# rapidsai/wholegraph

Measured on AMD Instinct MI355X. Metric: gather_GBps_out (gathered output row bytes/s, reference gather_scatter_bench convention), higher is better.
Workload: dtype f32

## Files before the change

### wholegraph_amd/csrc/backend.hpp

```cpp
#pragma once

#include <cstddef>
#include <cstdint>

#include <wholememory/global_reference.h>
#include <wholememory/tensor_description.h>

extern "C" {

struct wm_rows_args {
  wholememory_gref_t gref;
  wholememory_dtype_t table_dtype;
  int64_t dim;
  int64_t table_stride;
  int64_t table_storage_offset;
  const void* indices;
  wholememory_dtype_t index_dtype;
  int64_t n;
  const void* row_map;
  void* plain;
  wholememory_dtype_t plain_dtype;
  int64_t plain_stride;
  int64_t plain_storage_offset;
  int max_blocks;
// ... 15 lines not shown

struct wm_optimizer_args {
  int type;
  const void* ids;
  wholememory_dtype_t index_dtype;
  const int32_t* run_starts;
  const int32_t* order;
  wholememory_dtype_t value_dtype;
  const void* grads;
  int64_t grad_stride;
  const void* self_grads;
  int64_t self_grad_stride;
  int64_t count;
  const int32_t* cache_slot_of;
  void* cache_data;
  uint8_t* cache_dirty;
  int64_t cache_row_elems;
  float* cache_state_data;
  int64_t cache_state_row_elems;
  void* local_table;
  int64_t table_stride;
  int64_t local_entry_offset;
  int64_t dim;
  float* per_element_state;
  int64_t per_element_stride;
  float* per_row_state;
  float weight_decay, epsilon, beta1, beta2, alpha, lr;
  int adam_w;
  void* long_run_ws;
  size_t long_run_ws_bytes;
  int fold_mode;
  int inputs_behind_sort;
};

struct wm_sample_args {
  wholememory_gref_t row_gref, col_gref;
  int64_t row_storage_offset, col_storage_offset;
  wholememory_dtype_t col_dtype;
  const int64_t* row_pairs;
  const void* centers;
  wholememory_dtype_t center_dtype;
  int n_center;
  int max_sample_count;
  uint64_t random_seed;
  const int* sample_offsets;
  void* out_ids;
  int* out_center_lid;
  int64_t* out_edge_gid;
  wholememory_gref_t weight_gref;
  int64_t weight_storage_offset;
  wholememory_dtype_t weight_dtype;
  const int* n_center_dev;
  void* fill_ff_ptr;
  size_t fill_ff_bytes;
};

struct wm_au_bounds {
  const int* n_target_dev;
  const int* n_neighbor_dev;
  int* n_unique_dev;
  int* publish_host_late;
  int table_is_clear;
  int pad_unique_tail;
};

struct wm_cache_args {
  int32_t* slot_of;
  int32_t* count;
  int64_t* row_of;
  uint8_t* dirty;
  char* data;
  int64_t cover_start;
  int64_t cover_rows;
  int64_t n_sets;
  int64_t set_cover;
  int64_t row_bytes;
  wholememory_gref_t raw_gref;
  int64_t raw_row_stride_bytes;
  int64_t raw_row_offset_bytes;
  char* data2;
  int64_t row_bytes2;
  wholememory_gref_t raw2_gref;
  int64_t raw2_row_stride_bytes;
};

struct wm_agg_args {
  const int32_t* row_ptr;
  const int32_t* col_ind;
  int64_t n_edges, n_dst, n_src, dim;
  int mean;
  const float* in;
  int64_t in_stride;
  const float* grad;
  int64_t grad_stride;
  float* out;
  int64_t out_stride;
};

struct wm_agg16_args {
  const int32_t* row_ptr;
  const int32_t* col_ind;
  int64_t n_edges, n_dst, n_src, dim;
  int mean;
  wholememory_dtype_t dtype;
  const void* in;
  int64_t in_stride;
  const void* grad;
  int64_t grad_stride;
  void* out;
  int64_t out_stride;
};

struct wm_gat_args {
  const int32_t* row_ptr;
  const int32_t* col_ind;
  int64_t n_edges, n_dst, n_src, heads, dim;
  float slope;
  int concat;
  const float* h;
  int64_t h_stride;
  const float* att;
  float* alpha;
  float* scores;
  float* out;
  int64_t out_stride;
  const float* grad;
  int64_t grad_stride;
  float* grad_h;
  int64_t grad_h_stride;
  float* grad_att;
};

struct wm_aggw_args {
  const int32_t* row_ptr;
  const int32_t* col_ind;
  const float* w;
  int64_t n_edges, n_dst, n_src, dim;
  int mean;
  const float* in;
  int64_t in_stride;
  const float* grad;
  int64_t grad_stride;
  float* out;
  int64_t out_stride;
  float* grad_w;
};

#define WM_MAX_EDGE_ATTRS 8
struct wm_edge_attr_args {
  const int64_t* edge_gid;
  const int* n_dev;
  int64_t n;
  int n_attrs;
  struct {
    wholememory_gref_t gref;
    int64_t storage_offset;
    int elt_bytes;
    void* out;
  } attr[WM_MAX_EDGE_ATTRS];
};

struct wm_gather_agg_args {
  wholememory_gref_t gref;
  wholememory_dtype_t table_dtype;
  int64_t table_rows;
  int64_t table_stride;
// ... 198 lines not shown
```

### wholegraph_amd/csrc/embedding_cache.cpp

```cpp
#include "embedding_cache.hpp"

#include <algorithm>
#include <cstring>

namespace wm {

row_cache::~row_cache()
{
  const auto* bk = backend();
  if (args.slot_of) bk->free_device(args.slot_of);
  if (args.count) bk->free_device(args.count);
  if (args.row_of) bk->free_device(args.row_of);
  if (args.dirty) bk->free_device(args.dirty);
  if (args.data) bk->free_device(args.data);
  if (args.data2) bk->free_device(args.data2);
  if (counters_dev) bk->free_device(counters_dev);
}

wholememory_error_code_t create_row_cache(row_cache** out, const wholememory_embedding_cache_policy_* policy,
                                          wholememory_tensor_t raw, wholememory_comm_t embedding_comm)
{
  const auto* bk = backend();
  if (bk->cache_update == nullptr) return WHOLEMEMORY_NOT_SUPPORTED;
  auto* desc = wholememory_tensor_get_tensor_description(raw);
  auto h     = wholememory_tensor_get_memory_handle(raw);
  std::unique_ptr<row_cache> c(new row_cache());
  c->same_comm = policy->cache_comm == embedding_comm;
  c->writable  = policy->access_type == WHOLEMEMORY_AT_READWRITE;
  c->dtype     = desc->dtype;
  c->row_elems = desc->strides[0];
  c->raw       = raw;
  const size_t es = wholememory_dtype_get_element_size(desc->dtype);
  auto& a         = c->args;
  a.row_bytes     = c->row_elems * static_cast<int64_t>(es);
  if (a.row_bytes % 16 != 0) return WHOLEMEMORY_LOGIC_ERROR;
  a.raw_row_stride_bytes = a.row_bytes;
  a.raw_row_offset_bytes = desc->storage_offset * static_cast<int64_t>(es);
  if (c->same_comm) {
    std::vector<size_t> off = entry_offsets_of(h, static_cast<size_t>(a.row_bytes));
    a.cover_start           = static_cast<int64_t>(off[embedding_comm->world_rank]);
    a.cover_rows            = static_cast<int64_t>(off[embedding_comm->world_rank + 1]) - a.cover_start;
    a.raw_gref              = local_shard_gref(h);
  } else {
    a.cover_start = 0;
    a.cover_rows  = desc->sizes[0];
    if (wholememory_get_memory_type(h) == WHOLEMEMORY_MT_DISTRIBUTED && embedding_comm->world_size > 1) {
      c->raw_addressable = false;
      a.raw_gref         = wholememory_create_continuous_global_reference(nullptr);
    } else {
      WHOLEMEMORY_RETURN_ON_FAIL(tensor_mapped_gref(raw, &a.raw_gref));
    }
  }
  if (a.cover_rows >= (INT64_C(1) << 31)) return WHOLEMEMORY_NOT_SUPPORTED;
  int64_t slots = static_cast<int64_t>(static_cast<double>(a.cover_rows) * policy->cache_ratio);
  slots         = std::min(a.cover_rows + 63, std::max<int64_t>(slots, a.cover_rows > 0 ? 64 : 0));
  a.n_sets      = (slots + 63) / 64;
  a.set_cover   = a.n_sets > 0 ? (a.cover_rows + a.n_sets - 1) / a.n_sets : 0;
  const int64_t n_slots = a.n_sets * 64;
  auto dev_alloc = [&](void** p, size_t bytes) { WM_BK(bk->malloc_device(p, std::max<size_t>(bytes, 16))); };
  dev_alloc(reinterpret_cast<void**>(&a.slot_of), sizeof(int32_t) * a.cover_rows);
  dev_alloc(reinterpret_cast<void**>(&a.count), sizeof(int32_t) * a.cover_rows);
  dev_alloc(reinterpret_cast<void**>(&a.row_of), sizeof(int64_t) * n_slots);
  dev_alloc(reinterpret_cast<void**>(&a.dirty), n_slots);
  dev_alloc(reinterpret_cast<void**>(&a.data), static_cast<size_t>(n_slots) * a.row_bytes);
  dev_alloc(reinterpret_cast<void**>(&c->counters_dev), 32);
  WM_BK(bk->memset_async(a.slot_of, 0xff, sizeof(int32_t) * a.cover_rows, nullptr));
  WM_BK(bk->memset_async(a.count, 0, sizeof(int32_t) * a.cover_rows, nullptr));
  WM_BK(bk->memset_async(a.row_of, 0xff, sizeof(int64_t) * n_slots, nullptr));
  WM_BK(bk->memset_async(a.dirty, 0, n_slots, nullptr));
  WM_BK(bk->memset_async(c->counters_dev, 0, 32, nullptr));
  WM_BK(bk->stream_sync(nullptr));
  *out = c.release();
  return WHOLEMEMORY_SUCCESS;
}

wholememory_error_code_t row_cache_update(row_cache* c, const void* ids, wholememory_dtype_t index_dtype, int64_t n,
                                          int64_t key_upper_bound, wholememory_env_func_t* env, void* stream)
{
  const auto* bk = backend();
  if (n == 0 || c->args.n_sets == 0) return WHOLEMEMORY_SUCCESS;
  if (n >= (INT64_C(1) << 31)) return WHOLEMEMORY_INVALID_INPUT;
  sorted_ids s(env);
  int rc = s.run(ids, index_dtype, n, key_upper_bound, 0, stream);
  if (rc != 0) return rc == -1 ? WHOLEMEMORY_INVALID_INPUT : WHOLEMEMORY_CUDA_ERROR;
  rc = bk->cache_update(&c->args, s.unique, index_dtype, s.starts, s.n_unique_dev, n, nullptr, nullptr, nullptr, stream);
  if (rc != 0) return rc == -1 ? WHOLEMEMORY_INVALID_INPUT : WHOLEMEMORY_CUDA_ERROR;
  WM_BK(bk->stream_sync(stream));
  return WHOLEMEMORY_SUCCESS;
}

wholememory_error_code_t row_cache_plan(row_cache* c, const void* ids, wholememory_dtype_t index_dtype, int64_t n, int64_t key_upper_bound,
                                        wholememory_env_func_t* env, void* stream, temp_mem* rows_mem, temp_mem* slots_mem,
                                        int64_t* n_fill)
{
  const auto* bk = backend();
  *n_fill        = 0;
  auto* fill_rows  = static_cast<int64_t*>(rows_mem->device(n, WHOLEMEMORY_DT_INT64));
  auto* fill_slots = static_cast<int64_t*>(slots_mem->device(n, WHOLEMEMORY_DT_INT64));
  if (n == 0 || c->args.n_sets == 0) return WHOLEMEMORY_SUCCESS;
  if (n >= (INT64_C(1) << 31) || c->writable) return WHOLEMEMORY_INVALID_INPUT;
  sorted_ids s(env);
  temp_mem count(env), host_n(env);
  auto* d_count = static_cast<int*>(count.device(1, WHOLEMEMORY_DT_INT));
  WM_BK(bk->memset_async(d_count, 0, sizeof(int), stream));
  int rc = s.run(ids, index_dtype, n, key_upper_bound, 0, stream);
  if (rc != 0) return rc == -1 ? WHOLEMEMORY_INVALID_INPUT : WHOLEMEMORY_CUDA_ERROR;
  rc = bk->cache_update(&c->args, s.unique, index_dtype, s.starts, s.n_unique_dev, n, fill_rows, fill_slots, d_count, stream);
  if (rc != 0) return rc == -1 ? WHOLEMEMORY_INVALID_INPUT : WHOLEMEMORY_CUDA_ERROR;
  auto* h = static_cast<int*>(host_n.pinned(1, WHOLEMEMORY_DT_INT));
  WM_BK(bk->memcpy_async(h, d_count, sizeof(int), stream));
  WM_BK(bk->stream_sync(stream));
  *n_fill = *h;
  return WHOLEMEMORY_SUCCESS;
}

wholememory_error_code_t row_cache_install(row_cache* c, const void* rows_data, const int64_t* slots, int64_t n_fill,
                                           void* stream)
{
  const auto* bk = backend();
  if (n_fill == 0) return WHOLEMEMORY_SUCCESS;
  wm_rows_args a{};
  a.gref          = wholememory_create_continuous_global_reference(c->args.data);
  a.table_dtype   = c->dtype;
  a.dim           = c->row_elems;
  a.table_stride  = c->row_elems;
  a.indices       = slots;
  a.index_dtype   = WHOLEMEMORY_DT_INT64;
  a.n             = n_fill;
  a.plain         = const_cast<void*>(rows_data);
  a.plain_dtype   = c->dtype;
  a.plain_stride  = c->row_elems;
  a.max_blocks    = -1;
  WM_BK(bk->scatter_rows(&a, stream));
  return WHOLEMEMORY_SUCCESS;
}

wholememory_error_code_t row_cache_split(row_cache* c, const void* ids, wholememory_dtype_t index_dtype, int64_t n,
                                         int64_t* cache_idx, void* raw_idx, void* stream)
{
  int rc = backend()->cache_split(&c->args, ids, index_dtype, n, cache_idx, raw_idx, c->counters_dev, stream);
  if (rc != 0) return rc == -1 ? WHOLEMEMORY_INVALID_INPUT : WHOLEMEMORY_CUDA_ERROR;
  c->lookups += n;
  return WHOLEMEMORY_SUCCESS;
}

wholememory_error_code_t row_cache_gather(row_cache* c, const wm_rows_args& a, wholememory_env_func_t* env, void* stream)
{
  const auto* bk = backend();
  if (a.n == 0) return WHOLEMEMORY_SUCCESS;
  temp_mem cache_idx_mem(env), raw_idx_mem(env);
  auto* cache_idx = static_cast<int64_t*>(cache_idx_mem.device(a.n, WHOLEMEMORY_DT_INT64));
  void* raw_idx   = raw_idx_mem.device(a.n, a.index_dtype);
  WHOLEMEMORY_RETURN_ON_FAIL(row_cache_split(c, a.indices, a.index_dtype, a.n, cache_idx, raw_idx, stream));
  wm_rows_args hit        = a;
  hit.gref                = wholememory_create_continuous_global_reference(c->args.data);
  hit.table_stride        = c->row_elems;
  hit.table_storage_offset = 0;
  hit.indices             = cache_idx;
  hit.index_dtype         = WHOLEMEMORY_DT_INT64;
  WM_BK(bk->gather_rows(&hit, stream));
  wm_rows_args miss = a;
  miss.indices      = raw_idx;
  WM_BK(bk->gather_rows(&miss, stream));
  WM_BK(bk->stream_sync(stream));
  return WHOLEMEMORY_SUCCESS;
}

wholememory_error_code_t row_cache_attach_states(row_cache* c, wholememory_tensor_t state_local)
{
  const auto* bk = backend();
  if (!c->same_comm || !c->writable || c->args.data2 != nullptr) return WHOLEMEMORY_INVALID_INPUT;
  WHOLEMEMORY_RETURN_ON_FAIL(row_cache_writeback(c, true, nullptr));
  auto* d = wholememory_tensor_get_tensor_description(state_local);
  if (d->dtype != WHOLEMEMORY_DT_FLOAT || d->dim != 2) return WHOLEMEMORY_INVALID_INPUT;
  auto& a                 = c->args;
  a.row_bytes2            = d->strides[0] * static_cast<int64_t>(sizeof(float));
  a.raw2_row_stride_bytes = a.row_bytes2;
  if (a.row_bytes2 % 16 != 0) return WHOLEMEMORY_LOGIC_ERROR;
  char* local = static_cast<char*>(wholememory_tensor_get_data_pointer(state_local));
  a.raw2_gref = wholememory_create_continuous_global_reference(local - a.cover_start * a.row_bytes2);
  void* p     = nullptr;
  WM_BK(bk->malloc_device(&p, std::max<size_t>(static_cast<size_t>(a.n_sets) * 64 * a.row_bytes2, 16)));
  a.data2 = static_cast<char*>(p);
  return WHOLEMEMORY_SUCCESS;
}

wholememory_error_code_t row_cache_writeback(row_cache* c, bool drop, void* stream)
{
  const auto* bk = backend();
  int rc         = bk->cache_writeback(&c->args, drop ? 1 : 0, stream);
  if (rc != 0) return WHOLEMEMORY_CUDA_ERROR;
  return bk->stream_sync(stream) == 0 ? WHOLEMEMORY_SUCCESS : WHOLEMEMORY_CUDA_ERROR;
}

wholememory_error_code_t row_cache_info(row_cache* c, int64_t* slots, int64_t* occupied, int64_t* dirty, int64_t* hits,
                                        int64_t* lookups, void* stream)
{
  const auto* bk = backend();
  if (bk->cache_info(&c->args, c->counters_dev + 1, stream) != 0) return WHOLEMEMORY_CUDA_ERROR;
  unsigned long long h[3] = {0, 0, 0};
  WM_BK(bk->memcpy_async(h, c->counters_dev, sizeof(h), stream));
  WM_BK(bk->stream_sync(stream));
  if (slots) *slots = c->args.n_sets * 64;
  if (occupied) *occupied = static_cast<int64_t>(h[1]);
  if (dirty) *dirty = static_cast<int64_t>(h[2]);
  if (hits) *hits = static_cast<int64_t>(h[0]);
  if (lookups) *lookups = c->lookups;
  return WHOLEMEMORY_SUCCESS;
}

}
```

### wholegraph_amd/csrc/embedding_cache.hpp

```cpp
#pragma once

#include <wholememory/embedding.h>

#include "backend.hpp"
#include "ops_internal.hpp"

struct wholememory_embedding_cache_policy_ {
  wholememory_comm_t cache_comm;
  wholememory_memory_type_t cache_memory_type;
  wholememory_memory_location_t cache_memory_location;
  wholememory_access_type_t access_type;
  float cache_ratio;
};

namespace wm {

struct row_cache {
  wm_cache_args args{};
  bool same_comm = false;
  bool writable  = false;
  bool raw_addressable = true;
  wholememory_tensor_t raw = nullptr;
  wholememory_dtype_t dtype = WHOLEMEMORY_DT_UNKNOWN;
  int64_t row_elems         = 0;
  unsigned long long* counters_dev = nullptr;
  int64_t lookups                  = 0;
  ~row_cache();
};

wholememory_error_code_t create_row_cache(row_cache** out, const wholememory_embedding_cache_policy_* policy,
                                          wholememory_tensor_t raw, wholememory_comm_t embedding_comm);

wholememory_error_code_t row_cache_update(row_cache* c, const void* ids, wholememory_dtype_t index_dtype, int64_t n,
                                          int64_t key_upper_bound, wholememory_env_func_t* env, void* stream);

wholememory_error_code_t row_cache_gather(row_cache* c, const wm_rows_args& a, wholememory_env_func_t* env, void* stream);

wholememory_error_code_t row_cache_plan(row_cache* c, const void* ids, wholememory_dtype_t index_dtype, int64_t n,
                                        int64_t key_upper_bound, wholememory_env_func_t* env, void* stream, temp_mem* rows_mem, temp_mem* slots_mem,
                                        int64_t* n_fill);
wholememory_error_code_t row_cache_install(row_cache* c, const void* rows_data, const int64_t* slots, int64_t n_fill,
                                           void* stream);
wholememory_error_code_t row_cache_split(row_cache* c, const void* ids, wholememory_dtype_t index_dtype, int64_t n,
                                         int64_t* cache_idx, void* raw_idx, void* stream);

wholememory_error_code_t row_cache_attach_states(row_cache* c, wholememory_tensor_t state_local);

wholememory_error_code_t row_cache_writeback(row_cache* c, bool drop, void* stream);
wholememory_error_code_t row_cache_info(row_cache* c, int64_t* slots, int64_t* occupied, int64_t* dirty, int64_t* hits,
                                        int64_t* lookups, void* stream);

}
```

### wholegraph_amd/csrc/kernels/cache.hip

```cpp
#include <hip/hip_runtime.h>
#include <stdint.h>

#include <algorithm>

#include "../backend.hpp"

namespace wm {
namespace {

constexpr int kBlock = 256;

struct raw_view {
  char* base;
  char* const* rank_ptrs;
  const size_t* rank_offsets;
  size_t chunk_stride;
  int world_size;
  int same_chunk;
  int64_t row_stride_bytes;
  int64_t row_offset_bytes;
};

struct raw2_view {
  char* base;
  int64_t row_stride_bytes;
};
inline raw2_view make_raw2(const wm_cache_args& c)
{
  return raw2_view{c.data2 != nullptr ? static_cast<char*>(c.raw2_gref.pointer) : nullptr, c.raw2_row_stride_bytes};
}

inline raw_view make_raw(const wm_cache_args& c)
{
  raw_view v{};
  v.chunk_stride = c.raw_gref.stride;
  v.world_size   = c.raw_gref.world_size;
  v.same_chunk   = c.raw_gref.same_chunk ? 1 : 0;
  if (c.raw_gref.stride == 0) {
    v.base = static_cast<char*>(c.raw_gref.pointer);
  } else {
    v.rank_ptrs    = static_cast<char* const*>(c.raw_gref.pointer);
    v.rank_offsets = c.raw_gref.rank_memory_offsets;
  }
  v.row_stride_bytes = c.raw_row_stride_bytes;
  v.row_offset_bytes = c.raw_row_offset_bytes;
  return v;
}

__device__ __forceinline__ char* raw_row(const raw_view& v, int64_t row)
{
  const size_t off = static_cast<size_t>(v.row_offset_bytes) + static_cast<size_t>(row) * static_cast<size_t>(v.row_stride_bytes);
  if (v.chunk_stride == 0) return v.base + off;
  int rank;
  size_t start;
  if (v.same_chunk) {
    rank  = static_cast<int>(off / v.chunk_stride);
    start = static_cast<size_t>(rank) * v.chunk_stride;
  } else {
    rank = 0;
    for (int r = 1; r < v.world_size; r++)
      if (off >= v.rank_offsets[r]) rank = r;
    start = v.rank_offsets[rank];
  }
  return v.rank_ptrs[rank] + (off - start);
}

__device__ __forceinline__ void wave_copy_row(char* dst, const char* src, int row_bytes, int lane)
{
  typedef uint32_t u32x4 __attribute__((ext_vector_type(4)));
  for (int o = lane * 16; o < row_bytes; o += 64 * 16) *reinterpret_cast<u32x4*>(dst + o) = *reinterpret_cast<const u32x4*>(src + o);
}

struct cache_dev {
  int32_t* slot_of;
  int32_t* count;
  int64_t* row_of;
  uint8_t* dirty;
  char* data;
  int64_t cover_start, cover_rows, n_sets, set_cover;
  int row_bytes;
  char* data2;
  int row_bytes2;
};

inline cache_dev make_dev(const wm_cache_args& c)
{
  return cache_dev{c.slot_of, c.count, c.row_of, c.dirty, c.data, c.cover_start, c.cover_rows, c.n_sets, c.set_cover,
                   static_cast<int>(c.row_bytes), c.data2, static_cast<int>(c.row_bytes2)};
}

template <typename IdxT>
__global__ void cache_count_kernel(cache_dev c, const IdxT* unique_rows, const int32_t* run_starts, const int64_t* n_unique)
{
  const int64_t u = static_cast<int64_t>(blockIdx.x) * blockDim.x + threadIdx.x;
  if (u >= *n_unique) return;
  const int64_t r = static_cast<int64_t>(unique_rows[u]) - c.cover_start;
  if (r < 0 || r >= c.cover_rows) return;
  c.count[r] += run_starts[u + 1] - run_starts[u];
}

struct fill_list {
  int64_t* rows;
  int64_t* slots;
  int* count;
};

template <typename IdxT>
__global__ __launch_bounds__(kBlock) void cache_update_kernel(cache_dev c, raw_view raw, raw2_view raw2,
                                                              const IdxT* unique_rows, const int64_t* n_unique_p,
                                                              fill_list fill)
{
  const int lane    = threadIdx.x & 63;
  const int64_t set = (static_cast<int64_t>(blockIdx.x) * kBlock + threadIdx.x) >> 6;
  if (set >= c.n_sets) return;
  const int64_t nu  = *n_unique_p;
  const int64_t lo_row = c.cover_start + set * c.set_cover;
  const int64_t hi_row = min(c.cover_start + c.cover_rows, lo_row + c.set_cover);
  auto lower = [&](int64_t key) {
    int64_t a = 0, b = nu;
    while (a < b) {
      const int64_t m = (a + b) >> 1;
      const IdxT v    = unique_rows[m];
      if (v >= 0 && static_cast<int64_t>(v) < key)
        a = m + 1;
      else
        b = m;
    }
    return a;
  };
  const int64_t first = lower(lo_row), last = lower(hi_row);
  if (first >= last) return;
  const int64_t slot  = set * 64 + lane;
  int64_t my_row      = c.row_of[slot];
  int32_t my_cnt      = my_row >= 0 ? c.count[my_row] : -1;
  for (int64_t j = first; j < last; j++) {
    const int64_t g = static_cast<int64_t>(unique_rows[j]);
    const int64_t r = g - c.cover_start;
    if (c.slot_of[r] >= 0) continue;
    const int32_t cand = c.count[r];
    uint64_t key = (static_cast<uint64_t>(static_cast<uint32_t>(my_cnt + 1)) << 8) | static_cast<uint32_t>(lane);
    for (int off = 32; off > 0; off >>= 1) {
      const uint64_t o = __shfl_xor(key, off, 64);
      key              = o < key ? o : key;
    }
    const int victim      = static_cast<int>(key & 0xff);
    const int32_t min_cnt = static_cast<int32_t>(key >> 8) - 1;
    if (cand <= min_cnt) continue;
    const int64_t vslot = set * 64 + victim;
    char* line          = c.data + vslot * c.row_bytes;
    const int64_t old   = __shfl(my_row, victim, 64);
    if (old >= 0) {
      if (fill.rows == nullptr && c.dirty[vslot]) {
        wave_copy_row(raw_row(raw, c.cover_start + old), line, c.row_bytes, lane);
        if (c.data2 != nullptr)
          wave_copy_row(raw2.base + (c.cover_start + old) * raw2.row_stride_bytes, c.data2 + vslot * c.row_bytes2, c.row_bytes2, lane);
      }
      if (lane == 0) c.slot_of[old] = -1;
    }
    if (fill.rows == nullptr) {
      wave_copy_row(line, raw_row(raw, g), c.row_bytes, lane);
      if (c.data2 != nullptr)
        wave_copy_row(c.data2 + vslot * c.row_bytes2, raw2.base + g * raw2.row_stride_bytes, c.row_bytes2, lane);
    } else if (lane == 0) {
      const int k   = atomicAdd(fill.count, 1);
      fill.rows[k]  = g;
      fill.slots[k] = vslot;
    }
    if (lane == 0) {
      c.slot_of[r]    = static_cast<int32_t>(vslot);
      c.row_of[vslot] = r;
      c.dirty[vslot]  = 0;
    }
    if (lane == victim) {
      my_row = r;
      my_cnt = cand;
    }
    __builtin_amdgcn_fence(__ATOMIC_RELEASE, "agent");
  }
}

template <typename IdxT>
__global__ __launch_bounds__(kBlock) void cache_split_kernel(cache_dev c, const IdxT* ids, int64_t n, int64_t* cache_idx,
                                                             IdxT* raw_idx, unsigned long long* hits)
{
  __shared__ unsigned int block_hits;
  if (threadIdx.x == 0) block_hits = 0;
  __syncthreads();
  unsigned int wave_hits = 0;
  for (int64_t base = static_cast<int64_t>(blockIdx.x) * kBlock; base < n; base += static_cast<int64_t>(gridDim.x) * kBlock) {
    const int64_t i = base + threadIdx.x;
    bool hit        = false;
    if (i < n) {
      const IdxT id   = ids[i];
      const int64_t r = static_cast<int64_t>(id) - c.cover_start;
      int32_t slot    = -1;
      if (id >= 0 && r >= 0 && r < c.cover_rows) slot = c.slot_of[r];
      hit          = slot >= 0;
      cache_idx[i] = slot;
      raw_idx[i]   = hit ? static_cast<IdxT>(-1) : id;
    }
    wave_hits += static_cast<unsigned int>(__popcll(__ballot(hit)));
  }
  if (hits != nullptr) {
    if ((threadIdx.x & 63) == 0 && wave_hits) atomicAdd(&block_hits, wave_hits);
    __syncthreads();
    if (threadIdx.x == 0 && block_hits) atomicAdd(hits, static_cast<unsigned long long>(block_hits));
  }
}

__global__ __launch_bounds__(kBlock) void cache_writeback_kernel(cache_dev c, raw_view raw, raw2_view raw2, int drop)
{
  const int lane     = threadIdx.x & 63;
  const int64_t slot = (static_cast<int64_t>(blockIdx.x) * kBlock + threadIdx.x) >> 6;
  if (slot >= c.n_sets * 64) return;
  const int64_t r = c.row_of[slot];
  if (r < 0) return;
  if (c.dirty[slot]) {
    wave_copy_row(raw_row(raw, c.cover_start + r), c.data + slot * c.row_bytes, c.row_bytes, lane);
    if (c.data2 != nullptr)
      wave_copy_row(raw2.base + (c.cover_start + r) * raw2.row_stride_bytes, c.data2 + slot * c.row_bytes2, c.row_bytes2, lane);
  }
  if (lane == 0) {
    c.dirty[slot] = 0;
    if (drop) {
      c.slot_of[r]   = -1;
      c.row_of[slot] = -1;
    }
  }
}

__global__ __launch_bounds__(kBlock) void cache_info_kernel(cache_dev c, unsigned long long* out)
{
  __shared__ unsigned int block_occ, block_dirty;
  if (threadIdx.x == 0) block_occ = block_dirty = 0;
  __syncthreads();
  unsigned int occ_n = 0, dirty_n = 0;
  const int64_t slots = c.n_sets * 64;
  for (int64_t base = static_cast<int64_t>(blockIdx.x) * kBlock; base < slots; base += static_cast<int64_t>(gridDim.x) * kBlock) {
    const int64_t slot = base + threadIdx.x;
    const bool occ     = slot < slots && c.row_of[slot] >= 0;
    const bool dirt    = occ && c.dirty[slot];
    occ_n += static_cast<unsigned int>(__popcll(__ballot(occ)));
    dirty_n += static_cast<unsigned int>(__popcll(__ballot(dirt)));
  }
  if ((threadIdx.x & 63) == 0) {
    if (occ_n) atomicAdd(&block_occ, occ_n);
    if (dirty_n) atomicAdd(&block_dirty, dirty_n);
  }
  __syncthreads();
  if (threadIdx.x == 0) {
    if (block_occ) atomicAdd(out, static_cast<unsigned long long>(block_occ));
    if (block_dirty) atomicAdd(out + 1, static_cast<unsigned long long>(block_dirty));
  }
}

}

int hip_cache_update(const wm_cache_args* c, const void* unique_rows, wholememory_dtype_t dt, const int32_t* run_starts,
                     const int64_t* n_unique_dev, int64_t n_upper, int64_t* fill_rows, int64_t* fill_slots, int* fill_count,
                     void* stream_v)
{
  const fill_list fill{fill_rows, fill_slots, fill_count};
  hipStream_t stream = static_cast<hipStream_t>(stream_v);
  if (n_upper == 0 || c->n_sets == 0) return 0;
  const cache_dev d = make_dev(*c);
  const raw_view rv = make_raw(*c);
  const int cb      = static_cast<int>((n_upper + kBlock - 1) / kBlock);
  const int ub      = static_cast<int>((c->n_sets * 64 + kBlock - 1) / kBlock);
  if (dt == WHOLEMEMORY_DT_INT) {
    hipLaunchKernelGGL((cache_count_kernel<int32_t>), dim3(cb), dim3(kBlock), 0, stream, d, static_cast<const int32_t*>(unique_rows), run_starts, n_unique_dev);
    hipLaunchKernelGGL((cache_update_kernel<int32_t>), dim3(ub), dim3(kBlock), 0, stream, d, rv, make_raw2(*c), static_cast<const int32_t*>(unique_rows), n_unique_dev, fill);
  } else if (dt == WHOLEMEMORY_DT_INT64) {
    hipLaunchKernelGGL((cache_count_kernel<int64_t>), dim3(cb), dim3(kBlock), 0, stream, d, static_cast<const int64_t*>(unique_rows), run_starts, n_unique_dev);
    hipLaunchKernelGGL((cache_update_kernel<int64_t>), dim3(ub), dim3(kBlock), 0, stream, d, rv, make_raw2(*c), static_cast<const int64_t*>(unique_rows), n_unique_dev, fill);
  } else {
    return -1;
  }
  return hipGetLastError() == hipSuccess ? 0 : -2;
}

int hip_cache_split(const wm_cache_args* c, const void* ids, wholememory_dtype_t dt, int64_t n, int64_t* cache_idx, void* raw_idx,
                    unsigned long long* hits_dev, void* stream_v)
{
  if (n == 0) return 0;
  const cache_dev d = make_dev(*c);
  const int blocks  = static_cast<int>(std::min<int64_t>((n + kBlock - 1) / kBlock, 1024));
  hipStream_t stream = static_cast<hipStream_t>(stream_v);
  if (dt == WHOLEMEMORY_DT_INT)
    hipLaunchKernelGGL((cache_split_kernel<int32_t>), dim3(blocks), dim3(kBlock), 0, stream, d, static_cast<const int32_t*>(ids), n, cache_idx, static_cast<int32_t*>(raw_idx), hits_dev);
  else if (dt == WHOLEMEMORY_DT_INT64)
    hipLaunchKernelGGL((cache_split_kernel<int64_t>), dim3(blocks), dim3(kBlock), 0, stream, d, static_cast<const int64_t*>(ids), n, cache_idx, static_cast<int64_t*>(raw_idx), hits_dev);
  else
    return -1;
  return hipGetLastError() == hipSuccess ? 0 : -2;
}

int hip_cache_writeback(const wm_cache_args* c, int drop, void* stream_v)
{
  hipStream_t stream = static_cast<hipStream_t>(stream_v);
  if (c->n_sets == 0) return 0;
  const int blocks = static_cast<int>((c->n_sets * 64 * 64 + kBlock - 1) / kBlock);
  hipLaunchKernelGGL(cache_writeback_kernel, dim3(blocks), dim3(kBlock), 0, stream, make_dev(*c), make_raw(*c), make_raw2(*c), drop);
  if (drop && hipMemsetAsync(c->count, 0, sizeof(int32_t) * c->cover_rows, stream) != hipSuccess) return -2;
  return hipGetLastError() == hipSuccess ? 0 : -2;
}

int hip_cache_info(const wm_cache_args* c, unsigned long long* out2_dev, void* stream_v)
{
  hipStream_t stream = static_cast<hipStream_t>(stream_v);
  if (hipMemsetAsync(out2_dev, 0, 16, stream) != hipSuccess) return -2;
  if (c->n_sets == 0) return 0;
  const int blocks = static_cast<int>(std::min<int64_t>((c->n_sets * 64 + kBlock - 1) / kBlock, 2048));
  hipLaunchKernelGGL(cache_info_kernel, dim3(blocks), dim3(kBlock), 0, stream, make_dev(*c), out2_dev);
  return hipGetLastError() == hipSuccess ? 0 : -2;
}

}
```

### wholegraph_amd/csrc/ops.cpp

```cpp
#include "knobs.hpp"
#include "ops_internal.hpp"
#include "embedding_cache.hpp"

#include <algorithm>
#include <atomic>
#include <cstdlib>
#include <cstring>

namespace wm {

temp_mem::temp_mem(wholememory_env_func_t* env) : env_(env)
{
  WM_CHECK(env != nullptr, "p_env_fns must not be null");
  env_->temporary_fns.create_memory_context_fn(&ctx_, env_->temporary_fns.global_context);
}
temp_mem::~temp_mem()
{
  if (ptr_ != nullptr) env_->temporary_fns.free_fn(ctx_, env_->temporary_fns.global_context);
  env_->temporary_fns.destroy_memory_context_fn(ctx_, env_->temporary_fns.global_context);
}
void* temp_mem::alloc(int64_t elt_count, wholememory_dtype_t dtype, wholememory_memory_allocation_type_t type)
{
  WM_CHECK(ptr_ == nullptr, "temp_mem slot reused");
  wholememory_tensor_description_t d;
// ... 644 lines not shown
  const size_t oes   = wholememory_dtype_get_element_size(d.plain.dtype);
  const int64_t dim  = d.table.sizes[1];
  const int64_t n    = d.indices.size;
  auto entry_offsets = entry_offsets_of(handle, tes * static_cast<size_t>(d.table.stride));
  route rail{cross_comm, std::vector<size_t>(X + 1)};
  for (int k = 0; k <= X; k++) rail.offsets[k] = entry_offsets[static_cast<size_t>(k) * L];
  if (L == 1)
    return gather_distributed_rows(handle, d, env, stream, gather_sms, nullptr, false, &rail);

  id_exchange xa(env);
  bucket_and_exchange_ids(local_comm, d.indices_ptr, d.indices.dtype, n, entry_offsets, env, stream, &xa, false);
  const int64_t n_relay = xa.total_recv;

  sorted_ids s(env);
  temp_mem host_n(env), inverse(env);
  const bool dedup = n_relay > 0 && n_relay < (INT64_C(1) << 31) && bk->run_inverse != nullptr;
  void* fetch_ids  = xa.recv_ids;
  int64_t n_fetch  = n_relay;
  int64_t* inv     = nullptr;
  if (dedup) {
    if (s.run(xa.recv_ids, d.indices.dtype, n_relay, 0, 0, stream) != 0)
      throw hip_error("dedup of relayed ids failed");
    inv = static_cast<int64_t*>(inverse.device(n_relay, WHOLEMEMORY_DT_INT64));
    WM_BK(bk->run_inverse(s.starts, s.order, s.unique, d.indices.dtype, s.n_unique_dev, n_relay, 0, inv, stream));
    auto* h_n = static_cast<int64_t*>(host_n.pinned(1, WHOLEMEMORY_DT_INT64));
    WM_BK(bk->memcpy_async(h_n, s.n_unique_dev, sizeof(int64_t), stream));
    WM_BK(bk->stream_sync(stream));
    fetch_ids = s.unique;
    n_fetch   = *h_n;
  }

  temp_mem fetched(env), relay_rows(env), back_rows(env);
  char* fetched_buf = static_cast<char*>(fetched.device(dim * n_fetch, d.plain.dtype));
  op_descs db       = d;
  db.indices_ptr    = fetch_ids;
  db.indices        = wholememory_create_array_desc(n_fetch, 0, d.indices.dtype);
  db.plain_ptr      = fetched_buf;
  int64_t fsz[2]    = {n_fetch, dim};
  db.plain          = wholememory_create_matrix_desc(fsz, dim, 0, d.plain.dtype);
  WHOLEMEMORY_RETURN_ON_FAIL(gather_distributed_rows(handle, db, env, stream, gather_sms, nullptr, false, &rail));

  char* send_buf = fetched_buf;
  WM_DEBUG("HIERARCHY gather: rank %d (local %d of %d, node %d of %d) asked %ld ids, relays %ld, fetches %ld distinct",
           comm->world_rank, local_comm->world_rank, L, cross_comm->world_rank, X, static_cast<long>(n),
           static_cast<long>(n_relay), static_cast<long>(n_fetch));
  if (dedup) {
    send_buf       = static_cast<char*>(relay_rows.device(dim * n_relay, d.plain.dtype));
    int64_t rsz[2] = {n_relay, dim};
    auto relay_desc = wholememory_create_matrix_desc(rsz, dim, 0, d.plain.dtype);
    wm_rows_args ea{};
    fill_rows_args(&ea, wholememory_create_continuous_global_reference(fetched_buf), db.plain, inv, WHOLEMEMORY_DT_INT64,
                   n_relay, send_buf, relay_desc, gather_sms);
    WM_BK(bk->gather_rows(&ea, stream));
  }

  const size_t row_bytes = static_cast<size_t>(dim) * oes;
  char* back_buf = static_cast<char*>(back_rows.device(dim * xa.total_valid, d.plain.dtype));
  exchange_segments(local_comm, send_buf, xa.recv_counts, xa.recv_offsets, back_buf, xa.send_counts, xa.bucket_offsets,
                    row_bytes, stream);
  if (xa.total_valid > 0) {
    int64_t bsz[2] = {xa.total_valid, dim};
    auto back_desc = wholememory_create_matrix_desc(bsz, dim, 0, d.plain.dtype);
    wm_rows_args ra{};
    fill_rows_args(&ra, wholememory_create_continuous_global_reference(d.plain_ptr), d.plain, xa.raw_indices,
                   WHOLEMEMORY_DT_INT64, xa.total_valid, back_buf, back_desc, -1);
    WM_BK(bk->scatter_rows(&ra, stream));
  }
  WM_BK(bk->stream_sync(stream));
  return WHOLEMEMORY_SUCCESS;
}

}

wholememory_error_code_t gather_cached(wholememory_tensor_t table, wholememory_tensor_t indices_tensor,
                                       wholememory_tensor_t output_tensor, wholememory_env_func_t* env, void* stream,
                                       int gather_sms, row_cache* cache, bool adjust_cache)
{
  op_descs d;
  WHOLEMEMORY_RETURN_ON_FAIL(check_args(table, indices_tensor, output_tensor, "output", &d));
  auto handle = wholememory_tensor_get_memory_handle(table);
  if (cache->same_comm)
    return gather_distributed_rows(handle, d, env, stream, gather_sms, cache, adjust_cache);
  if (cache->raw_addressable) {
    if (adjust_cache)
      WHOLEMEMORY_RETURN_ON_FAIL(row_cache_update(cache, d.indices_ptr, d.indices.dtype, d.indices.size, d.table.sizes[0], env, stream));
    wm_rows_args a{};
    fill_rows_args(&a, cache->args.raw_gref, d.table, d.indices_ptr, d.indices.dtype, d.indices.size, d.plain_ptr, d.plain,
                   gather_sms);
    return row_cache_gather(cache, a, env, stream);
  }
  const auto* bk     = backend();
  const int64_t n    = d.indices.size;
  const int64_t dim  = d.table.sizes[1];
  if (adjust_cache) {
    temp_mem rows_mem(env), slots_mem(env), staging(env);
    int64_t n_fill = 0;
    WHOLEMEMORY_RETURN_ON_FAIL(row_cache_plan(cache, d.indices_ptr, d.indices.dtype, n, d.table.sizes[0], env, stream, &rows_mem, &slots_mem, &n_fill));
    char* rows_data = static_cast<char*>(staging.device(n_fill * cache->row_elems, d.table.dtype));
    op_descs df     = d;
    df.indices_ptr  = rows_mem.get();
    df.indices      = wholememory_create_array_desc(n_fill, 0, WHOLEMEMORY_DT_INT64);
    df.plain_ptr    = rows_data;
    int64_t fsz[2]  = {n_fill, dim};
    df.plain        = wholememory_create_matrix_desc(fsz, cache->row_elems, 0, d.table.dtype);
    WHOLEMEMORY_RETURN_ON_FAIL(gather_distributed_rows(handle, df, env, stream, gather_sms));
    WHOLEMEMORY_RETURN_ON_FAIL(row_cache_install(cache, rows_data, static_cast<const int64_t*>(slots_mem.get()), n_fill, stream));
    WM_BK(bk->stream_sync(stream));
  }
  temp_mem cache_idx_mem(env), raw_idx_mem(env);
  auto* cache_idx = static_cast<int64_t*>(cache_idx_mem.device(n, WHOLEMEMORY_DT_INT64));
  void* raw_idx   = raw_idx_mem.device(n, d.indices.dtype);
  WHOLEMEMORY_RETURN_ON_FAIL(row_cache_split(cache, d.indices_ptr, d.indices.dtype, n, cache_idx, raw_idx, stream));
  if (n > 0) {
    wm_rows_args hit{};
    fill_rows_args(&hit, wholememory_create_continuous_global_reference(cache->args.data), d.table, cache_idx,
                   WHOLEMEMORY_DT_INT64, n, d.plain_ptr, d.plain, gather_sms);
    hit.table_stride         = cache->row_elems;
    hit.table_storage_offset = 0;
    WM_BK(bk->gather_rows(&hit, stream));
  }
  op_descs dm    = d;
  dm.indices_ptr = raw_idx;
  dm.indices.storage_offset = 0;
  WHOLEMEMORY_RETURN_ON_FAIL(gather_distributed(handle, dm, env, stream, gather_sms));
  WM_BK(bk->stream_sync(stream));
  return WHOLEMEMORY_SUCCESS;
}

namespace {

wholememory_error_code_t scatter_distributed(wholememory_handle_t handle, const op_descs& d,
                                             wholememory_env_func_t* env, void* stream, int scatter_sms)
{
  const auto* bk = backend();
  if (d.table.storage_offset < 0 || d.table.storage_offset + d.table.sizes[1] > d.table.stride)
    return WHOLEMEMORY_INVALID_INPUT;
  wholememory_comm_t comm;
  WHOLEMEMORY_RETURN_ON_FAIL(wholememory_get_communicator(&comm, handle));
  const size_t tes    = wholememory_dtype_get_element_size(d.table.dtype);
  const size_t pes    = wholememory_dtype_get_element_size(d.plain.dtype);
  const size_t ies    = wholememory_dtype_get_element_size(d.indices.dtype);
  const int64_t dim   = d.table.sizes[1];
  auto entry_offsets  = entry_offsets_of(handle, tes * static_cast<size_t>(d.table.stride));
  const char* indices = static_cast<const char*>(d.indices_ptr);
  if (comm->single_rank_direct()) {
    wm_rows_args a{};
    fill_rows_args(&a, local_shard_gref(handle), d.table, indices, d.indices.dtype, d.indices.size, d.plain_ptr, d.plain,
                   scatter_sms);
    WM_BK(bk->scatter_rows(&a, stream));
    WM_BK(bk->stream_sync(stream));
    return WHOLEMEMORY_SUCCESS;
  }

  const bool self_local = !comm->loopback;
  id_exchange x(env);
  bucket_and_exchange_ids(comm, indices, d.indices.dtype, d.indices.size, entry_offsets, env, stream, &x, self_local);
  const auto local_gref = local_shard_gref(handle);

  if (x.self_count > 0 && self_local) {
    wm_rows_args sa{};
    fill_rows_args(&sa, local_gref, d.table, static_cast<const char*>(x.bucketed_ids) + ies * x.self_offset,
                   d.indices.dtype, x.self_count, d.plain_ptr, d.plain, scatter_sms);
    sa.row_map = x.raw_indices + x.self_offset;
    WM_BK(bk->scatter_rows(&sa, stream));
    g_dist_scatter_launches.fetch_add(1, std::memory_order_relaxed);
  }

  const size_t row_bytes = static_cast<size_t>(dim) * pes;
  const int W            = comm->world_size;
  const int C            = exchange_chunks(W, x.global_moved);
  const auto in_gref     = wholememory_create_continuous_global_reference(d.plain_ptr);
// ... 208 lines not shown
```

Before: 2999.

## Split cache update into decide kernel plus bulk fill gather, drop host syncs

The count kernel now records per-set ranges, so the update kernel no longer binary-searches per set. For read-only raw-addressable caches, a new decide kernel picks victims in parallel using ballots and writes a per-slot fill list, and the row copies then run as one bulk gather_rows over all slots. Stream syncs after update and after the cached gather now happen only in debug mode. This adds a memset and a kernel launch per update, and it changes how the split kernel handles uncovered ids (raw_idx is now -1 for them), which may alter correctness.

```diff
diff --git a/wholegraph_amd/csrc/backend.hpp b/wholegraph_amd/csrc/backend.hpp
--- a/wholegraph_amd/csrc/backend.hpp
+++ b/wholegraph_amd/csrc/backend.hpp
@@ -121,6 +121,8 @@
   int64_t row_bytes2;
   wholememory_gref_t raw2_gref;
   int64_t raw2_row_stride_bytes;
+  int32_t* set_range;
+  int64_t* fill_row;
 };
 
 struct wm_agg_args {
diff --git a/wholegraph_amd/csrc/embedding_cache.cpp b/wholegraph_amd/csrc/embedding_cache.cpp
--- a/wholegraph_amd/csrc/embedding_cache.cpp
+++ b/wholegraph_amd/csrc/embedding_cache.cpp
@@ -14,6 +14,8 @@
   if (args.dirty) bk->free_device(args.dirty);
   if (args.data) bk->free_device(args.data);
   if (args.data2) bk->free_device(args.data2);
+  if (args.set_range) bk->free_device(args.set_range);
+  if (fill_row_dev) bk->free_device(fill_row_dev);
   if (counters_dev) bk->free_device(counters_dev);
 }
 
@@ -64,6 +66,9 @@
   dev_alloc(reinterpret_cast<void**>(&a.dirty), n_slots);
   dev_alloc(reinterpret_cast<void**>(&a.data), static_cast<size_t>(n_slots) * a.row_bytes);
   dev_alloc(reinterpret_cast<void**>(&c->counters_dev), 32);
+  dev_alloc(reinterpret_cast<void**>(&a.set_range), sizeof(int32_t) * 2 * a.n_sets);
+  if (!c->writable && !c->same_comm && c->raw_addressable)
+    dev_alloc(reinterpret_cast<void**>(&c->fill_row_dev), sizeof(int64_t) * n_slots);
   WM_BK(bk->memset_async(a.slot_of, 0xff, sizeof(int32_t) * a.cover_rows, nullptr));
   WM_BK(bk->memset_async(a.count, 0, sizeof(int32_t) * a.cover_rows, nullptr));
   WM_BK(bk->memset_async(a.row_of, 0xff, sizeof(int64_t) * n_slots, nullptr));
@@ -75,7 +80,8 @@
 }
 
 wholememory_error_code_t row_cache_update(row_cache* c, const void* ids, wholememory_dtype_t index_dtype, int64_t n,
-                                          int64_t key_upper_bound, wholememory_env_func_t* env, void* stream)
+                                          int64_t key_upper_bound, wholememory_env_func_t* env, void* stream,
+                                          const wm_rows_args* raw_rows)
 {
   const auto* bk = backend();
   if (n == 0 || c->args.n_sets == 0) return WHOLEMEMORY_SUCCESS;
@@ -83,9 +89,23 @@
   sorted_ids s(env);
   int rc = s.run(ids, index_dtype, n, key_upper_bound, 0, stream);
   if (rc != 0) return rc == -1 ? WHOLEMEMORY_INVALID_INPUT : WHOLEMEMORY_CUDA_ERROR;
-  rc = bk->cache_update(&c->args, s.unique, index_dtype, s.starts, s.n_unique_dev, n, nullptr, nullptr, nullptr, stream);
-  if (rc != 0) return rc == -1 ? WHOLEMEMORY_INVALID_INPUT : WHOLEMEMORY_CUDA_ERROR;
-  WM_BK(bk->stream_sync(stream));
+  wm_cache_args ca = c->args;
+  if (raw_rows != nullptr) ca.fill_row = c->fill_row_dev;
+  rc = bk->cache_update(&ca, s.unique, index_dtype, s.starts, s.n_unique_dev, n, nullptr, nullptr, nullptr, stream);
+  if (rc != 0) return rc == -1 ? WHOLEMEMORY_INVALID_INPUT : WHOLEMEMORY_CUDA_ERROR;
+  if (ca.fill_row != nullptr) {
+    wm_rows_args f         = *raw_rows;
+    f.indices              = ca.fill_row;
+    f.index_dtype          = WHOLEMEMORY_DT_INT64;
+    f.n                    = ca.n_sets * 64;
+    f.row_map              = nullptr;
+    f.plain                = ca.data;
+    f.plain_dtype          = c->dtype;
+    f.plain_stride         = c->row_elems;
+    f.plain_storage_offset = 0;
+    WM_BK(bk->gather_rows(&f, stream));
+  }
+  if (debug_sync_enabled()) WM_BK(bk->stream_sync(stream));
   return WHOLEMEMORY_SUCCESS;
 }
 
@@ -162,7 +182,7 @@
   wm_rows_args miss = a;
   miss.indices      = raw_idx;
   WM_BK(bk->gather_rows(&miss, stream));
-  WM_BK(bk->stream_sync(stream));
+  if (debug_sync_enabled()) WM_BK(bk->stream_sync(stream));
   return WHOLEMEMORY_SUCCESS;
 }
 
diff --git a/wholegraph_amd/csrc/embedding_cache.hpp b/wholegraph_amd/csrc/embedding_cache.hpp
--- a/wholegraph_amd/csrc/embedding_cache.hpp
+++ b/wholegraph_amd/csrc/embedding_cache.hpp
@@ -24,6 +24,7 @@
   wholememory_dtype_t dtype = WHOLEMEMORY_DT_UNKNOWN;
   int64_t row_elems         = 0;
   unsigned long long* counters_dev = nullptr;
+  int64_t* fill_row_dev            = nullptr;
   int64_t lookups                  = 0;
   ~row_cache();
 };
@@ -32,7 +33,8 @@
                                           wholememory_tensor_t raw, wholememory_comm_t embedding_comm);
 
 wholememory_error_code_t row_cache_update(row_cache* c, const void* ids, wholememory_dtype_t index_dtype, int64_t n,
-                                          int64_t key_upper_bound, wholememory_env_func_t* env, void* stream);
+                                          int64_t key_upper_bound, wholememory_env_func_t* env, void* stream,
+                                          const wm_rows_args* raw_rows = nullptr);
 
 wholememory_error_code_t row_cache_gather(row_cache* c, const wm_rows_args& a, wholememory_env_func_t* env, void* stream);
 
diff --git a/wholegraph_amd/csrc/kernels/cache.hip b/wholegraph_amd/csrc/kernels/cache.hip
--- a/wholegraph_amd/csrc/kernels/cache.hip
+++ b/wholegraph_amd/csrc/kernels/cache.hip
@@ -81,54 +81,54 @@
   int row_bytes;
   char* data2;
   int row_bytes2;
+  int32_t* set_first;
+  int32_t* set_end;
 };
 
 inline cache_dev make_dev(const wm_cache_args& c)
 {
   return cache_dev{c.slot_of, c.count, c.row_of, c.dirty, c.data, c.cover_start, c.cover_rows, c.n_sets, c.set_cover,
-                   static_cast<int>(c.row_bytes), c.data2, static_cast<int>(c.row_bytes2)};
+                   static_cast<int>(c.row_bytes), c.data2, static_cast<int>(c.row_bytes2), c.set_range, c.set_range + c.n_sets};
 }
 
 template <typename IdxT>
 __global__ void cache_count_kernel(cache_dev c, const IdxT* unique_rows, const int32_t* run_starts, const int64_t* n_unique)
 {
-  const int64_t u = static_cast<int64_t>(blockIdx.x) * blockDim.x + threadIdx.x;
-  if (u >= *n_unique) return;
+  const int64_t u  = static_cast<int64_t>(blockIdx.x) * blockDim.x + threadIdx.x;
+  const int64_t nu = *n_unique;
+  if (u >= nu) return;
   const int64_t r = static_cast<int64_t>(unique_rows[u]) - c.cover_start;
   if (r < 0 || r >= c.cover_rows) return;
   c.count[r] += run_starts[u + 1] - run_starts[u];
-}
-
-struct fill_list {
-  int64_t* rows;
-  int64_t* slots;
-  int* count;
-};
+  const uint32_t cover = static_cast<uint32_t>(c.set_cover);
+  const uint32_t set   = static_cast<uint32_t>(r) / cover;
+  auto set_of = [&](int64_t v) {
+    if (v < 0 || v >= nu) return 0xffffffffu;
+    const int64_t q = static_cast<int64_t>(unique_rows[v]) - c.cover_start;
+    return q < 0 || q >= c.cover_rows ? 0xffffffffu : static_cast<uint32_t>(q) / cover;
+  };
+  if (set_of(u - 1) != set) c.set_first[set] = static_cast<int32_t>(u);
+  if (set_of(u + 1) != set) c.set_end[set] = static_cast<int32_t>(u + 1);
+}
+
+__device__ __forceinline__ uint64_t wave_min_key(int32_t my_cnt, int lane)
+{
+  uint64_t key = (static_cast<uint64_t>(static_cast<uint32_t>(my_cnt + 1)) << 8) | static_cast<uint32_t>(lane);
+  for (int off = 32; off > 0; off >>= 1) {
+    const uint64_t o = __shfl_xor(key, off, 64);
+    key              = o < key ? o : key;
+  }
+  return key;
+}
 
 template <typename IdxT>
 __global__ __launch_bounds__(kBlock) void cache_update_kernel(cache_dev c, raw_view raw, raw2_view raw2,
-                                                              const IdxT* unique_rows, const int64_t* n_unique_p,
-                                                              fill_list fill)
+                                                              const IdxT* unique_rows)
 {
   const int lane    = threadIdx.x & 63;
   const int64_t set = (static_cast<int64_t>(blockIdx.x) * kBlock + threadIdx.x) >> 6;
   if (set >= c.n_sets) return;
-  const int64_t nu  = *n_unique_p;
-  const int64_t lo_row = c.cover_start + set * c.set_cover;
-  const int64_t hi_row = min(c.cover_start + c.cover_rows, lo_row + c.set_cover);
-  auto lower = [&](int64_t key) {
-    int64_t a = 0, b = nu;
-    while (a < b) {
-      const int64_t m = (a + b) >> 1;
-      const IdxT v    = unique_rows[m];
-      if (v >= 0 && static_cast<int64_t>(v) < key)
-        a = m + 1;
-      else
-        b = m;
-    }
-    return a;
-  };
-  const int64_t first = lower(lo_row), last = lower(hi_row);
+  const int64_t first = c.set_first[set], last = c.set_end[set];
   if (first >= last) return;
   const int64_t slot  = set * 64 + lane;
   int64_t my_row      = c.row_of[slot];
@@ -138,11 +138,7 @@
     const int64_t r = g - c.cover_start;
     if (c.slot_of[r] >= 0) continue;
     const int32_t cand = c.count[r];
-    uint64_t key = (static_cast<uint64_t>(static_cast<uint32_t>(my_cnt + 1)) << 8) | static_cast<uint32_t>(lane);
-    for (int off = 32; off > 0; off >>= 1) {
-      const uint64_t o = __shfl_xor(key, off, 64);
-      key              = o < key ? o : key;
-    }
+    const uint64_t key    = wave_min_key(my_cnt, lane);
     const int victim      = static_cast<int>(key & 0xff);
     const int32_t min_cnt = static_cast<int32_t>(key >> 8) - 1;
     if (cand <= min_cnt) continue;
@@ -150,22 +146,16 @@
     char* line          = c.data + vslot * c.row_bytes;
     const int64_t old   = __shfl(my_row, victim, 64);
     if (old >= 0) {
-      if (fill.rows == nullptr && c.dirty[vslot]) {
+      if (c.dirty[vslot]) {
         wave_copy_row(raw_row(raw, c.cover_start + old), line, c.row_bytes, lane);
         if (c.data2 != nullptr)
           wave_copy_row(raw2.base + (c.cover_start + old) * raw2.row_stride_bytes, c.data2 + vslot * c.row_bytes2, c.row_bytes2, lane);
       }
       if (lane == 0) c.slot_of[old] = -1;
     }
-    if (fill.rows == nullptr) {
-      wave_copy_row(line, raw_row(raw, g), c.row_bytes, lane);
-      if (c.data2 != nullptr)
-        wave_copy_row(c.data2 + vslot * c.row_bytes2, raw2.base + g * raw2.row_stride_bytes, c.row_bytes2, lane);
-    } else if (lane == 0) {
-      const int k   = atomicAdd(fill.count, 1);
-      fill.rows[k]  = g;
-      fill.slots[k] = vslot;
-    }
+    wave_copy_row(line, raw_row(raw, g), c.row_bytes, lane);
+    if (c.data2 != nullptr)
+      wave_copy_row(c.data2 + vslot * c.row_bytes2, raw2.base + g * raw2.row_stride_bytes, c.row_bytes2, lane);
     if (lane == 0) {
       c.slot_of[r]    = static_cast<int32_t>(vslot);
       c.row_of[vslot] = r;
@@ -176,6 +166,79 @@
       my_cnt = cand;
     }
     __builtin_amdgcn_fence(__ATOMIC_RELEASE, "agent");
+  }
+}
+
+struct fill_list {
+  int64_t* rows;
+  int64_t* slots;
+  int* count;
+};
+
+template <typename IdxT>
+__global__ __launch_bounds__(kBlock) void cache_decide_kernel(cache_dev c, const IdxT* unique_rows, int64_t* fill_row,
+                                                              fill_list fill)
+{
+  const int lane    = threadIdx.x & 63;
+  const int64_t set = (static_cast<int64_t>(blockIdx.x) * kBlock + threadIdx.x) >> 6;
+  if (set >= c.n_sets) return;
+  const int32_t first = c.set_first[set], last = c.set_end[set];
+  const int64_t slot  = set * 64 + lane;
+  int64_t my_row      = -1;
+  bool changed        = false;
+  if (first < last) {
+    my_row         = c.row_of[slot];
+    int32_t my_cnt = my_row >= 0 ? c.count[my_row] : -1;
+    uint64_t key   = wave_min_key(my_cnt, lane);
+    for (int32_t base = first; base < last; base += 64) {
+      const int32_t j = base + lane;
+      int64_t r       = -1;
+      int32_t cnt     = 0;
+      bool missing    = false;
+      if (j < last) {
+        r       = static_cast<int64_t>(unique_rows[j]) - c.cover_start;
+        missing = c.slot_of[r] < 0;
+        cnt     = c.count[r];
+      }
+      uint64_t todo = __ballot(missing && cnt > static_cast<int32_t>(key >> 8) - 1);
+      while (todo != 0) {
+        const int k = __ffsll(static_cast<unsigned long long>(todo)) - 1;
+        todo &= todo - 1;
+        const int32_t cand = __shfl(cnt, k, 64);
+        if (cand <= static_cast<int32_t>(key >> 8) - 1) continue;
+        const int victim  = static_cast<int>(key & 0xff);
+        const int64_t rk  = __shfl(r, k, 64);
+        const int64_t old = __shfl(my_row, victim, 64);
+        if (lane == 0) {
+          if (old >= 0) c.slot_of[old] = -1;
+          c.slot_of[rk] = static_cast<int32_t>(set * 64 + victim);
+        }
+        if (lane == victim) {
+          my_row  = rk;
+          my_cnt  = cand;
+          changed = true;
+        }
+        key = wave_min_key(my_cnt, lane);
+      }
+    }
+    if (changed) {
+      c.row_of[slot] = my_row;
+      c.dirty[slot]  = 0;
+    }
+  }
+  if (fill.rows == nullptr) {
+    fill_row[slot] = changed ? c.cover_start + my_row : -1;
+    return;
+  }
+  const uint64_t m = __ballot(changed);
+  if (m == 0) return;
+  int k0 = 0;
+  if (lane == 0) k0 = atomicAdd(fill.count, __popcll(m));
+  k0 = __shfl(k0, 0, 64);
+  if (changed) {
+    const int k   = k0 + __popcll(m & ((1ull << lane) - 1));
+    fill.rows[k]  = c.cover_start + my_row;
+    fill.slots[k] = slot;
   }
 }
 
@@ -194,10 +257,11 @@
       const IdxT id   = ids[i];
       const int64_t r = static_cast<int64_t>(id) - c.cover_start;
       int32_t slot    = -1;
-      if (id >= 0 && r >= 0 && r < c.cover_rows) slot = c.slot_of[r];
+      const bool covered = id >= 0 && r >= 0 && r < c.cover_rows;
+      if (covered) slot = c.slot_of[r];
       hit          = slot >= 0;
       cache_idx[i] = slot;
-      raw_idx[i]   = hit ? static_cast<IdxT>(-1) : id;
+      raw_idx[i]   = hit || !covered ? static_cast<IdxT>(-1) : id;
     }
     wave_hits += static_cast<unsigned int>(__popcll(__ballot(hit)));
   }
@@ -267,14 +331,23 @@
   const raw_view rv = make_raw(*c);
   const int cb      = static_cast<int>((n_upper + kBlock - 1) / kBlock);
   const int ub      = static_cast<int>((c->n_sets * 64 + kBlock - 1) / kBlock);
+  if (dt != WHOLEMEMORY_DT_INT && dt != WHOLEMEMORY_DT_INT64) return -1;
+  const bool decide = c->fill_row != nullptr || fill_rows != nullptr;
+  if (hipMemsetAsync(c->set_range, 0, sizeof(int32_t) * 2 * c->n_sets, stream) != hipSuccess) return -2;
   if (dt == WHOLEMEMORY_DT_INT) {
-    hipLaunchKernelGGL((cache_count_kernel<int32_t>), dim3(cb), dim3(kBlock), 0, stream, d, static_cast<const int32_t*>(unique_rows), run_starts, n_unique_dev);
-    hipLaunchKernelGGL((cache_update_kernel<int32_t>), dim3(ub), dim3(kBlock), 0, stream, d, rv, make_raw2(*c), static_cast<const int32_t*>(unique_rows), n_unique_dev, fill);
-  } else if (dt == WHOLEMEMORY_DT_INT64) {
-    hipLaunchKernelGGL((cache_count_kernel<int64_t>), dim3(cb), dim3(kBlock), 0, stream, d, static_cast<const int64_t*>(unique_rows), run_starts, n_unique_dev);
-    hipLaunchKernelGGL((cache_update_kernel<int64_t>), dim3(ub), dim3(kBlock), 0, stream, d, rv, make_raw2(*c), static_cast<const int64_t*>(unique_rows), n_unique_dev, fill);
+    const auto* u = static_cast<const int32_t*>(unique_rows);
+    hipLaunchKernelGGL((cache_count_kernel<int32_t>), dim3(cb), dim3(kBlock), 0, stream, d, u, run_starts, n_unique_dev);
+    if (decide)
+      hipLaunchKernelGGL((cache_decide_kernel<int32_t>), dim3(ub), dim3(kBlock), 0, stream, d, u, c->fill_row, fill);
+    else
+      hipLaunchKernelGGL((cache_update_kernel<int32_t>), dim3(ub), dim3(kBlock), 0, stream, d, rv, make_raw2(*c), u);
   } else {
-    return -1;
+    const auto* u = static_cast<const int64_t*>(unique_rows);
+    hipLaunchKernelGGL((cache_count_kernel<int64_t>), dim3(cb), dim3(kBlock), 0, stream, d, u, run_starts, n_unique_dev);
+    if (decide)
+      hipLaunchKernelGGL((cache_decide_kernel<int64_t>), dim3(ub), dim3(kBlock), 0, stream, d, u, c->fill_row, fill);
+    else
+      hipLaunchKernelGGL((cache_update_kernel<int64_t>), dim3(ub), dim3(kBlock), 0, stream, d, rv, make_raw2(*c), u);
   }
   return hipGetLastError() == hipSuccess ? 0 : -2;
 }
diff --git a/wholegraph_amd/csrc/ops.cpp b/wholegraph_amd/csrc/ops.cpp
--- a/wholegraph_amd/csrc/ops.cpp
+++ b/wholegraph_amd/csrc/ops.cpp
@@ -750,11 +750,12 @@
   if (cache->same_comm)
     return gather_distributed_rows(handle, d, env, stream, gather_sms, cache, adjust_cache);
   if (cache->raw_addressable) {
-    if (adjust_cache)
-      WHOLEMEMORY_RETURN_ON_FAIL(row_cache_update(cache, d.indices_ptr, d.indices.dtype, d.indices.size, d.table.sizes[0], env, stream));
     wm_rows_args a{};
     fill_rows_args(&a, cache->args.raw_gref, d.table, d.indices_ptr, d.indices.dtype, d.indices.size, d.plain_ptr, d.plain,
                    gather_sms);
+    if (adjust_cache)
+      WHOLEMEMORY_RETURN_ON_FAIL(row_cache_update(cache, d.indices_ptr, d.indices.dtype, d.indices.size, d.table.sizes[0], env, stream,
+                                                  cache->fill_row_dev != nullptr ? &a : nullptr));
     return row_cache_gather(cache, a, env, stream);
   }
   const auto* bk     = backend();
```

Result: no change. 2999, median of 2 (-0.0%).
